# mikkleini/slam.net

Hardware: AMD Instinct MI355X
Metric: candidate-pose distance evals/sec on 2048^2 map, 1080-ray scan, 1/2/4/8 GPU (higher is better)
Workload: dtype f32 transform + u16 gather / integer sum

## Files before the change

slam.net_amd/csrc/cs_internal.h:

```cpp
#pragma once
#include "common.h"
#include <time.h>
#include <stdio.h>
#include <stdlib.h>
#include <vector>
#include <utility>

#define CS_RB_MAX 64
#define CS_RB_EXTENT_PX 128.0f
#define K1_GROUP 1024
#define K1_GROUP_BIG 2048
#define K1_RING_SLOTS 4
#define K1_GROUP_SMALL 512
#define K1_PLAN_SLOTS 8


struct k1_block_term { double a, b, m, n, nr; };

struct slamhip_cs {
    slamhip_ctx *ctx;
    float physical;
    int hs; float hscale;
    int os; float oscale;
    uint16_t *d_hole;
// ... 31 lines not shown
    bool gen_pending; uint64_t gen_seed, gen_stream;
    int shard_first, shard_count;
    float *d_ev_off;
    int *d_ev_idx;
    int cap_cand;
    float4 *d_pxcs;
    void *d_partial; size_t cap_partial;
    unsigned long long *d_k1_gmin;
    unsigned long long *d_k1_acc;
    int k1_cap_groups;
    int k1_group;
    std::vector<float> h_grp_dth, h_grp_dxy;
    std::vector<float> h_grp_lohi;
    std::vector<int> k1_tab_group, k1_tab_nc, k1_tab_nbp; int k1_uni_g0, k1_uni_ng, k1_uni_nc;
    std::vector<k1_block_term> k1_terms; std::vector<double> k1_cost, k1_lc; std::vector<int> k1_share;
    std::vector<std::pair<int, std::vector<int>>> k1_cut_cache; uint32_t k1_cut_gen, k1_cut_layout_gen;
    float k1_last_pose[3]; bool k1_last_valid;
    uint32_t k1_cut_seen_scan, k1_cut_seen_layout;
    uint32_t k1_layout_gen;
    std::vector<char> k1_cut_cand;
    std::vector<double> k1_cut_wsc;
    std::vector<double> k1_cut_wb;
    uint32_t scan_gen;
    std::vector<float> h_grp_prev; int k1_group_prev;
    bool k1_layout_dirty, k1_layout_spread; int k1_layout_budget, k1_layout_groups; float k1_layout_theta;
    bool k1_scan_dirty;
    bool k1_prelaunch;
    uint64_t pl_stats[4];
    uint32_t *d_scan_flag; uint32_t scan_flag_seq;
    bool k1_layout_stale;
    int k1_layout_target;
    float gen_sigma_xy, gen_sigma_theta;
    bool offs_theta_small;
    unsigned int *d_verify;
    int32_t *d_dist;
    uint64_t *d_key;
    uint64_t *h_key;
    float *d_grp_bounds; int cap_grp;
    float *d_best_pose;
    bool k1_want_pose;
    bool k1_pose_written;
    unsigned *k1_done_flag; unsigned k1_done_val;
    bool k1_done_armed;
    unsigned long long *k1_sig; unsigned long long k1_sig_val; bool k1_sig_armed;
    uint64_t *d_k1_ring; unsigned k1_ring_pos, k1_ring_rested;
    bool ov_op_dirty, ov_side_unjoined;
    hipEvent_t ev_ov_op, ev_ov_side;
    bool k1_ring_request;
    bool k1_ring_may_overlap;
    uint64_t *k1_ring_last;
    hipStream_t plan_stream;
    uint2 *d_plan_rec[K1_PLAN_SLOTS];
    int plan_cap_wgs;
    uint32_t plan_seq;
    uint32_t plan_count;
    uint32_t k1_launches;
    int k1_last_stream;
    uint32_t k1_cross_no[2];
    uint32_t plan_slot_user[K1_PLAN_SLOTS];
    uint8_t plan_slot_stream[K1_PLAN_SLOTS];
    uint32_t plan_inputs_after;
    uint64_t plan_stats[4];
    void *d_rep; uint32_t *h_rep; uint32_t rep_seq;
    bool k1_keep_dist;
    bool rep_dist_valid; int rep_K;
    uint32_t upload_seq;

    void *d_rays; int cap_rays;
    void *d_k2_cand;
    void *d_k2_vprof;
    int *d_k2_start;
    int *d_k2_counters;
    void *mirror_reg; size_t mirror_reg_bytes;
    bool mirror_on, mirror_pending;
    int2 *d_hole_span, *d_hole_span_snap;
    uint16_t *d_hole_shadow;
    unsigned long long *d_mirror_mask; int mirror_chunks;
    int *d_mirror_sum; int *h_mirror_sum;
    hipStream_t mirror_stream; hipEvent_t ev_snap, ev_push;
    void *mirror_dev_ptr;
    unsigned mirror_reg_flags;
    uint16_t *mirror_user; bool mirror_direct;
    uint16_t *h_mirror_stage;
    int2 *d_mirror_rows, *h_mirror_rows;
    int *d_hole_dirty;
    int64_t last_hole_pixels;
    bool hole_pixels_pending;

    uint32_t *d_o_hits[2];
    uint8_t *d_o_nohit[2];
    int obst_buf;
    bool obst_pending; int obst_pend_buf, obst_pend_max_hits;
};

int32_t cs_alloc_candidates(slamhip_cs *cs, int count);
int32_t cs_plan_drain(slamhip_cs *cs);
void    cs_plan_free(slamhip_cs *cs);
static inline void cs_plan_inputs_pending(slamhip_cs *cs) { cs->plan_inputs_after = cs->k1_launches + 1; cs->ov_op_dirty = true; }
int32_t cs_overlap_join(slamhip_cs *cs);
int32_t cs_flush_scan(slamhip_cs *cs);
int32_t cs_launch_distance(slamhip_cs *cs, int mode, const float pose[3], int count, bool want_dist, bool cand_sane,
                           uint64_t *key_dst);
#define CS_REP_WORDS 30
#define CS_REP_KEY 30
#define CS_REP_POSE 32
#define CS_REP_FLAG 63
// ... 54 lines not shown
```

slam.net_amd/csrc/distance.hip:

```cpp
#include "cs_internal.h"
#include "det_trig.h"
#include <stdlib.h>
#include <algorithm>

#define K1_THREADS 256

__device__ static inline void k1_coords(const float4 q, const float2 p, float &fx, float &fy)
{
    fx = q.x + q.z * p.x;  fx = fx - q.w * p.y;
    fy = q.y + q.w * p.x;  fy = fy + q.z * p.y;
}

template <bool SAFE>
__device__ static inline void k1_gather_global(const uint16_t *__restrict__ map, int S, const float4 q, const float2 p,
                                               uint32_t &sum, uint32_t &cnt)
{
    float fx, fy;
    k1_coords(q, p, fx, fy);
    int ix, iy;
    if (SAFE) { ix = sh_f2i(fx); iy = sh_f2i(fy); }
    else      { ix = (int)fx;    iy = (int)fy; }
    const bool ok = ((unsigned)ix < (unsigned)S) & ((unsigned)iy < (unsigned)S);
    uint32_t v = 0;
    if (ok) v = map[(size_t)iy * S + ix];
// ... 108 lines not shown
        __syncthreads();
    }
    if (w == 0) {
        for (int off = 32; off > 0; off >>= 1) {
            const unsigned long long o = __shfl_down(key, off, 64);
            key = o < key ? o : key;
        }
        if (lane == 0 && key != ~0ull) atomicMin(key_out, key);
    }
}

#define K1_KIND_SHARED 1
#define K1_KIND_GLOBAL 2
#define K1_KIND_BAND 3
#define K1_MAXP 16
#define K1_MAXR 512
#define K1_MAXBANDS 4
#define K1_MAXSTEPS (K1_MAXP * K1_MAXBANDS * 2)
static_assert(K1_MAXBANDS == 4, "the step threads split t into (piece, band) with shifts");
#define K1_TABLE_G 64
#define K1_TABLE_WGS 2048
#define K1_MAXCUT 596
#define K1_ACC_INMAP 36
#define K1_ACC_ARRIVED 50
#define K1_ZERO_OFS 0
#define K1_TILE_OFS 16

struct k1_args {
    const uint16_t *map; int S;
    const float2 *pts;
    const int4 *ray_blk;
    int n_rays;
    const float4 *pxcs;
    const float *src3;
    float bx, by, bth, scale;
    int count, n_groups;
    int budget;
    int noden;
    int nopad;
    int nosplit;
    float band_stage;
    unsigned long long *acc;
    unsigned long long *gmin;
    unsigned *done;
    const int *ev_idx;
    int32_t *dist_out;
    unsigned long long *key_out;
    unsigned *verify;
    const float *offs_flat; float *best_pose;
    unsigned long long *sig; unsigned long long sig_val;
    unsigned *done_flag; unsigned done_val;
    unsigned long long *ring_slot, *ring_reset;
    uint2 *plan_rec; uint32_t plan_seq;
    uint32_t *started; uint32_t launch_no;
    const uint32_t *scan_flag; uint32_t scan_seq;
    int n_tab_wgs, uni_g0, uni_ng, uni_nc;
    int uni_cut, tab_cut;
    const float *grp_bounds;
    struct tab_rec {
        unsigned short group;
        unsigned short nbp;
        unsigned short first, nc;
    } tab[K1_TABLE_G];
    alignas(4) unsigned char wg_pos[K1_TABLE_WGS];
    alignas(4) unsigned short cut[K1_MAXCUT];
};
static_assert(sizeof(k1_args) <= 4096, "kernel arguments are limited to 4 KB");
static_assert(sizeof(k1_args::tab_rec) == 8 && offsetof(k1_args, tab) % 8 == 0, "table records are 8-byte aligned");
#define K1_PLAN_STEPS 15
#define K1_PLAN_REC_WORDS 128

#ifdef K1_TIMES
__device__ unsigned long long g_k1_times[4096 * 16];
__device__ unsigned long long g_k1_wstart[4096 * 16];
__device__ unsigned long long g_k1_sub[4096 * 8];
#define K1_SUB(k, v) { if (threadIdx.x == 0 && blockIdx.x < 4096) g_k1_sub[blockIdx.x * 8 + (k)] += (v); }
#define K1_STAMP(k) { if (threadIdx.x == 0 && blockIdx.x < 4096) g_k1_times[blockIdx.x * 16 + (k)] = wall_clock64(); }
#else
#define K1_STAMP(k) {}
#endif

__device__ static inline unsigned k1_tile_addr(int ix, int iy, int pitch2, int kofs)
{
    unsigned t, a;
    asm("v_lshl_add_u32 %0, %1, 1, %2" : "=v"(t) : "v"(ix), "s"(kofs));
    asm("v_mad_u32_u24 %0, %1, %2, %3" : "=v"(a) : "v"(iy), "s"(pitch2), "v"(t));
    return a;
}
__device__ static inline float k1_den(int v) { return __uint_as_float(v < 0 ? (0x80000000u | (unsigned)(-v)) : (unsigned)v); }
__device__ static inline unsigned k1_tile_addr_d(float fx, float fy, float two_d, float pitch2_d, float c_d)
{
    const float g = fmaf(truncf(fy), pitch2_d, fmaf(truncf(fx), two_d, c_d));
    return __float_as_uint(g);
}
typedef __attribute__((address_space(3))) const uint16_t k1_lds_u16;
__device__ static inline uint32_t k1_lds_load(unsigned addr) { return *(k1_lds_u16 *)(size_t)addr; }
typedef __attribute__((address_space(3))) const float k1_lds_f;
__device__ static inline float2 k1_point_lds(unsigned lds_addr)
{
    k1_lds_f *p = (k1_lds_f *)(size_t)lds_addr;
    return make_float2(p[0], p[1]);
}

typedef float k1_f32x4a8 __attribute__((ext_vector_type(4), aligned(8)));
__device__ static inline float4 k1_points2_lds(unsigned lds_addr)
{
// ... 144 lines not shown
    int zv;
    asm volatile("v_mov_b32 %0, 0" : "=v"(zv));
    const int wv = __builtin_amdgcn_readfirstlane(t >> 6);
    const k1_wg_t W = k1_wg_decode(a, (int)blockIdx.x);
    const int g = W.g, nc = W.nc, nbp = W.nbp;
    if (a.ring_reset && blockIdx.x == 0 && t == 0)
        __hip_atomic_store(a.ring_reset, ~0ull, __ATOMIC_RELAXED, __HIP_MEMORY_SCOPE_AGENT);
    if (a.started && blockIdx.x == 0 && t == 0)
        __hip_atomic_store(a.started, a.launch_no, __ATOMIC_RELAXED, __HIP_MEMORY_SCOPE_SYSTEM);
    K1_STAMP(0)
#ifdef K1_TIMES
    if (t == 0 && blockIdx.x < 4096) { for (int k = 0; k < 8; k++) g_k1_sub[blockIdx.x * 8 + k] = 0; }
    if (t == 0 && blockIdx.x < 4096) { for (int k = 10; k < 16; k++) g_k1_times[blockIdx.x * 16 + k] = 0; g_k1_times[blockIdx.x * 16 + 14] = (unsigned long long)g; g_k1_times[blockIdx.x * 16 + 15] = (unsigned long long)nc; }
    if (lane == 0 && blockIdx.x < 4096) g_k1_wstart[blockIdx.x * 16 + (wv & 15)] = wall_clock64();
    if (t == 0 && blockIdx.x < 4096) {
        unsigned hw, xcc;
        asm volatile("s_getreg_b32 %0, hwreg(HW_REG_HW_ID)" : "=s"(hw));
        asm volatile("s_getreg_b32 %0, hwreg(HW_REG_XCC_ID)" : "=s"(xcc));
        g_k1_wstart[blockIdx.x * 16 + 15] = ((unsigned long long)(xcc & 15u) << 16) | ((hw >> 8) & 0xffu);
    }
#endif
    const int bp = W.bp, rlo = W.rlo, rhi = W.rhi;
    const int nrays = rhi - rlo;
    if (a.scan_flag) {
        uint32_t v = 0;
        if (wv == 0) {
            int spins = 0;
            for (;;) {
                v = __hip_atomic_load(a.scan_flag, __ATOMIC_RELAXED, __HIP_MEMORY_SCOPE_SYSTEM);
                if ((v & 0x7fffffffu) == a.scan_seq) break;
                if (++spins > (1 << 23)) { if (t == 0) atomicAdd(a.verify, 1u); v = 0x80000000u; break; }
                __builtin_amdgcn_s_sleep(32);
            }
            if (blockIdx.x == 0 && t == 0) { ((uint32_t *)a.scan_flag)[8] = (uint32_t)spins; ((uint32_t *)a.scan_flag)[9] += (uint32_t)spins; }
            if (lane == 0) s_plan_ok = (int)v;
        }
        __syncthreads();
        v = (uint32_t)s_plan_ok;
        __syncthreads();
        if (__builtin_amdgcn_readfirstlane(v) & 0x80000000u) return;
    }
    const int blk_first = a.ray_blk[rlo + zv].z;
    const int blk_last_v = a.ray_blk[rhi - 1 + zv].z;

    const bool pre = MODE == 1 && a.grp_bounds != nullptr;
    float gb[6];
    if (pre) {
#pragma unroll
        for (int k = 0; k < 6; k++) gb[k] = a.grp_bounds[8 * (size_t)g + k];
    }
    const bool planned = MODE == 1 && !LAT && pre && a.plan_rec != nullptr;
    uint2 prw = make_uint2(0u, 0u);
    if (planned && wv == 0) prw = a.plan_rec[(size_t)blockIdx.x * (K1_PLAN_REC_WORDS / 2) + lane];
    float4 q[CPL];
    float c3[CPL][3];
#pragma unroll
    for (int k = 0; k < CPL; k++) {
        const int j = g * GROUP + k * LANES + t;
        const int jc = j < count ? j : count - 1;
        if (MODE == 0) q[k] = a.pxcs[jc];
        else { c3[k][0] = a.src3[3 * jc]; c3[k][1] = a.src3[3 * jc + 1]; c3[k][2] = a.src3[3 * jc + 2]; }
    }
    int4 rinfo[RU];
    float2 rpt[RU];
#pragma unroll
    for (int u = 0; u < RU; u++) {
        const int i = u * LANES + t;
        const int r = rlo + (i < nrays ? i : 0);
        rinfo[u] = make_int4(0, 0, 0, 0); rpt[u] = make_float2(0.f, 0.f);
        if (i < nrays) { rinfo[u] = a.ray_blk[r]; rpt[u] = a.pts[r]; }
    }
    if (t == 0) { s_nsteps = 0; s_plan_ok = 0; *(unsigned *)(smem + K1_ZERO_OFS) = 0u; }
    if (MODE != 0 && !pre) {
#pragma unroll
        for (int k = 0; k < CPL; k++) q[k] = k1_candidate<MODE == 0 ? 1 : MODE, true>(c3[k], a.bx, a.by, a.bth, a.scale);
    }
#pragma unroll
    for (int u = 0; u < RU; u++) {
        const int i = u * LANES + t;
        if (i < nrays) {
            cpts[i] = rpt[u];
            if (i == 0 || rinfo[u].x == rlo + i)
                pieces[rinfo[u].z - blk_first] = make_int2(i, (rinfo[u].y < rhi ? rinfo[u].y : rhi) - (rlo + i));
        }
    }
    bool have_plan = false;
    if (planned) {
        if (wv == 0) {
            const bool okl = ((lane & 3) != 3 || prw.y == a.plan_seq) && (lane != 0 || prw.x == a.plan_seq);
            const int ns = __builtin_amdgcn_readfirstlane((int)prw.y);
            const bool ok = __builtin_amdgcn_ballot_w64(okl) == ~0ull && ns >= 0 && ns <= K1_PLAN_STEPS;
            if (lane >= 4) *(int2 *)&stepbuf[2 * lane - 8] = make_int2((int)prw.x, (int)prw.y);
            if (lane == 0 && ok) { s_plan_ok = 1; s_nsteps = ns; }
        }
        __syncthreads();
        have_plan = __builtin_amdgcn_readfirstlane(s_plan_ok) != 0;
        if (VERIFY && t == 0) atomicAdd(a.verify + (have_plan ? 5 : 6), 1u);
    }
    K1_STAMP(1)
    if (!have_plan) {
    if (pre) {
        if (wv == 0) {
            k1_bounds_from_jitter(a, gb, bnd, lane);
        }
        __syncthreads();
        K1_STAMP(2)
    } else
    {
        float lo[4] = { q[0].x, q[0].y, q[0].z, q[0].w }, hi[4] = { q[0].x, q[0].y, q[0].z, q[0].w };
#pragma unroll
        for (int k = 1; k < CPL; k++) {
            lo[0] = fminf(lo[0], q[k].x); hi[0] = fmaxf(hi[0], q[k].x); lo[1] = fminf(lo[1], q[k].y); hi[1] = fmaxf(hi[1], q[k].y);
            lo[2] = fminf(lo[2], q[k].z); hi[2] = fmaxf(hi[2], q[k].z); lo[3] = fminf(lo[3], q[k].w); hi[3] = fmaxf(hi[3], q[k].w);
        }
        const float m0 = k1_wave_redf<false>(lo[0]), m1 = k1_wave_redf<true>(hi[0]);
        const float m2 = k1_wave_redf<false>(lo[1]), m3 = k1_wave_redf<true>(hi[1]);
        const float m4 = k1_wave_redf<false>(lo[2]), m5 = k1_wave_redf<true>(hi[2]);
        const float m6 = k1_wave_redf<false>(lo[3]), m7 = k1_wave_redf<true>(hi[3]);
        if (lane == 63) {
            *(float4 *)&wred[wv][0] = make_float4(m0, m1, m2, m3);
            *(float4 *)&wred[wv][4] = make_float4(m4, m5, m6, m7);
        }
        __syncthreads();
        K1_STAMP(2)
        if (t < 8) {
            float v[NW];
#pragma unroll
            for (int w = 0; w < NW; w++) v[w] = wred[w][t];
            float x = v[0];
#pragma unroll
            for (int w = 1; w < NW; w++) x = (t & 1) ? fmaxf(x, v[w]) : fminf(x, v[w]);
            bnd[t] = x;
        }
        __syncthreads();
    }
    K1_STAMP(3)
    const int npieces = __builtin_amdgcn_readfirstlane(blk_last_v - blk_first + 1);
#define K1_PIECE_STAMP K1_STAMP(4)
#define K1_STEP_SLOT(i) (i)
#define K1_PIECE_RAY(i) (i)
#include "k1_pieces.inc"
#undef K1_PIECE_RAY
#undef K1_STEP_SLOT
#undef K1_PIECE_STAMP
    __syncthreads();
    }
#ifdef K1_TIMES
    else if (t == 0 && blockIdx.x < 4096) { const unsigned long long now_ = wall_clock64(); for (int k = 2; k <= 4; k++) g_k1_times[blockIdx.x * 16 + k] = now_; }
#endif
    const int nsteps = s_nsteps;
// ... 16 lines not shown
        {                                                                                           \
             \
             \
             \
            const int4 pa_ = *(const int4 *)&stepbuf[(step) * 8];                                   \
            const int shift_ = __builtin_amdgcn_readfirstlane(stepbuf[(step) * 8 + 4]);             \
            const int w8_ = __builtin_amdgcn_readfirstlane(pa_.z), h_ = (enable) ? __builtin_amdgcn_readfirstlane(pa_.w) : 0; \
            const int rpi = 64 >> shift_;                          \
            const int srow = lane >> shift_, scol = lane & ((1 << shift_) - 1);                     \
            const bool colok = scol < (w8_ >> 3);                                                   \
            const int cc = colok ? scol : 0;                                                        \
            const unsigned S2_ = (unsigned)S * 2u;                                                  \
            const unsigned gofs = ((unsigned)__builtin_amdgcn_readfirstlane(pa_.y) * (unsigned)S + (unsigned)__builtin_amdgcn_readfirstlane(pa_.x)) * 2u; \
            const int pitchb = w8_ << 1;                                                            \
            const int row0 = wv * rpi + srow, rstep = NW * rpi;                                     \
            unsigned vofs = gofs + (unsigned)row0 * S2_ + ((unsigned)cc << 4);                      \
            int ldsd = K1_TILE_OFS + (cc << 4) + row0 * pitchb;                                     \
            const unsigned vstep = (unsigned)rstep * S2_;                                           \
            const int lstep = rstep * pitchb;                                                       \
            _Pragma("unroll") for (int k_ = 0; k_ < PF; k_++) {                                     \
                const bool live = colok & (row0 + k_ * rstep < h_);                                 \
                if (live && K1_EXP != 3) R[k_] = *(const k1_u32x4 *)((const char *)map + vofs);    \
                dst[k_] = live ? ldsd : -1;                                                         \
                vofs += vstep; ldsd += lstep;                                                       \
            }                                                                                       \
        }
#if K1_DMA0
        {
            const int4 pa_ = *(const int4 *)&stepbuf[0];
            const int w8_ = __builtin_amdgcn_readfirstlane(pa_.z), h_ = __builtin_amdgcn_readfirstlane(pa_.w);
            const int ncols = w8_ >> 3, nunits = ncols * h_;
            const unsigned S2_ = (unsigned)S * 2u;
            const unsigned gofs = ((unsigned)__builtin_amdgcn_readfirstlane(pa_.y) * (unsigned)S + (unsigned)__builtin_amdgcn_readfirstlane(pa_.x)) * 2u;
            const float rn = 1.0f / (float)ncols;
#pragma unroll
            for (int k_ = 0; k_ < PF; k_++) {
                const int e0 = (k_ * NW + wv) * 64;
                if (e0 < nunits && K1_EXP != 3) {
                    const int e = e0 + lane;
                    const int row = (int)(((float)e + 0.5f) * rn);
                    const int col = e - row * ncols;
                    if (e < nunits)
                        __builtin_amdgcn_global_load_lds((const __attribute__((address_space(1))) void *)((const char *)map + (gofs + (unsigned)row * S2_ + ((unsigned)col << 4))),
                                                         (__attribute__((address_space(3))) void *)(smem + K1_TILE_OFS + (e0 << 4)), 16, 0, 0);
                }
            }
#pragma unroll
            for (int k_ = 0; k_ < PF; k_++) dst[k_] = -1;
        }
#else
        K1_PREFETCH(0, true)
#endif
        if (MODE != 0 && pre) {
            {
#pragma unroll
            for (int k = 0; k < CPL; k++) { if (K1_EXP == 1) q[k] = make_float4(a.bx * a.scale + c3[k][0], a.by * a.scale + c3[k][1], a.scale, c3[k][2]); else q[k] = k1_candidate<MODE == 0 ? 1 : MODE, true>(c3[k], a.bx, a.by, a.bth, a.scale); }
            }
            if (LAT) {
#pragma unroll
                for (int k = 1; k < CPL; k++)
                    if (g * GROUP + k * LANES + t < count && (__float_as_uint(q[k].z) != __float_as_uint(q[0].z) || __float_as_uint(q[k].w) != __float_as_uint(q[0].w)))
                        atomicAdd(a.verify, 1u);
            }
        }
#ifdef K1_TIMES
        const unsigned long long sclk0 = clock64();
#endif
        for (int s = 0; s < nsteps; s++) {
#ifdef K1_TIMES
            const unsigned long long ts0 = wall_clock64();
#endif
            if (K1_DMA0 && s == 0) asm volatile("s_waitcnt vmcnt(0)" ::: "memory");
            else {
            __syncthreads();
#pragma unroll
            for (int k = 0; k < PF; k++) asm volatile("" : "+v"(R[k]));
#pragma unroll
            for (int k = 0; k < PF; k++) if (dst[k] >= 0 && K1_EXP != 3) *(k1_u32x4 *)(smem + dst[k]) = R[k];
            }
            __syncthreads();
            if (s == 0) K1_STAMP(6)
#ifdef K1_TIMES
            const unsigned long long ts1 = wall_clock64();
            if (s > 0) K1_SUB(0, ts1 - ts0)
#endif
            const int4 ca = *(const int4 *)&stepbuf[s * 8], cb = *(const int4 *)&stepbuf[s * 8 + 4];
            {
                const int sn = s + 1 < nsteps ? s + 1 : s;
                K1_PREFETCH(sn, s + 1 < nsteps)
            }
#ifdef K1_TIMES
            const unsigned long long ts2 = wall_clock64();
            K1_SUB(1, ts2 - ts1) K1_SUB(3, 1ull)
#endif
            const int kind = __builtin_amdgcn_readfirstlane(cb.y);
            const int nr = __builtin_amdgcn_readfirstlane(cb.z) >> 16;
#ifdef K1_TIMES
            if (t == 0 && blockIdx.x < 4096) g_k1_times[blockIdx.x * 16 + 10 + kind] += (unsigned long long)nr;
            if (t == 0 && blockIdx.x < 4096 && s < 3)
                g_k1_sub[blockIdx.x * 8 + 5 + s] = (unsigned long long)kind | ((unsigned long long)__builtin_amdgcn_readfirstlane(ca.z) << 4) | ((unsigned long long)__builtin_amdgcn_readfirstlane(ca.w) << 16) | ((unsigned long long)nr << 32);
#endif
            const unsigned pbase = cpts_lds + (unsigned)zv + (unsigned)(__builtin_amdgcn_readfirstlane(cb.z) & 0xffff) * 8u;
            const int x0a = __builtin_amdgcn_readfirstlane(ca.x), y0 = __builtin_amdgcn_readfirstlane(ca.y);
            const int w8 = __builtin_amdgcn_readfirstlane(ca.z), h = __builtin_amdgcn_readfirstlane(ca.w);
            const int pitch2 = w8 << 1;
            const int kofs = (int)smem_lds + K1_TILE_OFS - ((y0 * w8 + x0a) << 1);
            const unsigned zaddr = smem_lds + K1_ZERO_OFS + (unsigned)zv;
// ... 251 lines not shown
        __hip_atomic_store(a.done_flag, a.done_val, __ATOMIC_RELEASE, __HIP_MEMORY_SCOPE_SYSTEM);
    }
    K1_STAMP(9)
}


__device__ static inline int k1_plan_slot(const int i) { return i <= K1_PLAN_STEPS ? i : K1_PLAN_STEPS + 1; }
template <int GROUP, int CPL>
__global__ void __launch_bounds__(64)
k1_plan(const k1_args a, const int n_wgs)
{
    constexpr int NW = 1, PF = 64;
    const int lane = threadIdx.x, wv = 0;
    const uint32_t seq = a.plan_seq;
    if ((int)blockIdx.x >= n_wgs) return;
    __shared__ __attribute__((aligned(16))) int stepbuf[(K1_PLAN_STEPS + 2) * 8];
    __shared__ int2 pieces[K1_MAXP];
    __shared__ __attribute__((aligned(16))) float bnd[8];
    __shared__ int s_nsteps;
    const int S = a.S;
    const k1_wg_t W = k1_wg_decode(a, (int)blockIdx.x);
    const int g = W.g, nbp = W.nbp, bp = W.bp, rlo = W.rlo, rhi = W.rhi, nrays = rhi - rlo;
    float gb[6];
#pragma unroll
    for (int k = 0; k < 6; k++) gb[k] = a.grp_bounds[8 * (size_t)g + k];
    const int blk_first = a.ray_blk[rlo].z, blk_last = a.ray_blk[rhi - 1].z;
    if (lane == 0) s_nsteps = 0;
    for (int i = lane; i < nrays; i += 64) {
        const int4 ri = a.ray_blk[rlo + i];
        const int pidx = ri.z - blk_first;
        if ((i == 0 || ri.x == rlo + i) && (unsigned)pidx < (unsigned)K1_MAXP) pieces[pidx] = make_int2(i, (ri.y < rhi ? ri.y : rhi) - (rlo + i));
    }
    const float2 *cpts = a.pts + rlo;
    k1_bounds_from_jitter(a, gb, bnd, lane);
    __syncthreads();
    const int npieces = min(blk_last - blk_first + 1, K1_MAXP);
#define K1_PIECE_STAMP
#define K1_STEP_SLOT(i) k1_plan_slot(i)
#define K1_PIECE_RAY(i) min(max((i), 0), nrays - 1)
#include "k1_pieces.inc"
#undef K1_PIECE_RAY
#undef K1_STEP_SLOT
#undef K1_PIECE_STAMP
    __syncthreads();
    const int nsteps = s_nsteps;
    const bool fits = nsteps <= K1_PLAN_STEPS;
    const int unit = lane >> 2, wp = lane & 3;
    uint2 w = make_uint2(0u, 0u);
    if (unit > 0 && fits && unit - 1 < nsteps) { w.x = (uint32_t)stepbuf[(unit - 1) * 8 + 2 * wp]; w.y = (uint32_t)stepbuf[(unit - 1) * 8 + 2 * wp + 1]; }
    if (lane == 0) { w.x = seq; w.y = (uint32_t)(fits ? nsteps : -1); }
    if (wp == 3) w.y = seq;
    __hip_atomic_store((unsigned long long *)(a.plan_rec + (size_t)blockIdx.x * (K1_PLAN_REC_WORDS / 2) + lane), ((unsigned long long)w.y << 32) | w.x,
                       __ATOMIC_RELAXED, __HIP_MEMORY_SCOPE_AGENT);
}

int32_t cs_overlap_join(slamhip_cs *cs)
{
    cs->ov_op_dirty = true;
    if (!cs->ov_side_unjoined) return SLAMHIP_OK;
    if (!cs->ev_ov_side) SH_HIP(hipEventCreateWithFlags(&cs->ev_ov_side, hipEventDisableTiming));
    SH_HIP(hipEventRecord(cs->ev_ov_side, cs->side_stream));
    SH_HIP(hipStreamWaitEvent(cs->ctx->stream, cs->ev_ov_side, 0));
    cs->ov_side_unjoined = false;
    cs->k1_cross_no[1] = cs->k1_launches + 1;
    return SLAMHIP_OK;
}

int32_t cs_plan_drain(slamhip_cs *cs)
{
    if (cs->plan_stream) SH_HIP(hipStreamSynchronize(cs->plan_stream));
    return SLAMHIP_OK;
}

void cs_plan_free(slamhip_cs *cs)
{
    if (cs->plan_stream) (void)hipStreamSynchronize(cs->plan_stream);
    for (int i = 0; i < K1_PLAN_SLOTS; i++) {
        (void)hipFree(cs->d_plan_rec[i]);
        cs->d_plan_rec[i] = nullptr; cs->plan_slot_user[i] = 0;
    }
    cs->plan_cap_wgs = 0;
}

int32_t cs_alloc_candidates(slamhip_cs *cs, int count)
{
    if (count <= cs->cap_cand) return SLAMHIP_OK;
    SH_TRY(cs_plan_drain(cs));
    int cap = count + (count >> 2) + 256;
    if (cs->d_ev_off) (void)hipFree(cs->d_ev_off);
    if (cs->d_ev_idx) (void)hipFree(cs->d_ev_idx);
    if (cs->d_pxcs) (void)hipFree(cs->d_pxcs);
    if (cs->d_dist) (void)hipFree(cs->d_dist);
    cs->d_ev_off = nullptr; cs->d_ev_idx = nullptr; cs->d_pxcs = nullptr; cs->d_dist = nullptr; cs->cap_cand = 0;
    SH_HIP(hipMalloc(&cs->d_ev_off, sizeof(float) * 3 * (size_t)cap));
    SH_HIP(hipMalloc(&cs->d_ev_idx, sizeof(int) * (size_t)cap));
    SH_HIP(hipMalloc(&cs->d_pxcs, sizeof(float4) * (size_t)cap));
    SH_HIP(hipMalloc(&cs->d_dist, sizeof(int32_t) * (size_t)cap));
    if (cs->d_grp_bounds) (void)hipFree(cs->d_grp_bounds);
    cs->d_grp_bounds = nullptr; cs->cap_grp = 0;
    SH_HIP(hipMalloc(&cs->d_grp_bounds, sizeof(float) * 8 * (size_t)(cap / K1_GROUP_SMALL + 2)));
    cs->cap_grp = cap / K1_GROUP_SMALL + 2;
    cs->cap_cand = cap;
    cs->rep_dist_valid = false;
    cs->shard_first = -1; cs->shard_count = -1;
    return SLAMHIP_OK;
}

static int32_t ensure_partial(slamhip_cs *cs, size_t bytes)
{
    if (bytes <= cs->cap_partial) return SLAMHIP_OK;
    if (cs->d_partial) (void)hipFree(cs->d_partial);
    cs->d_partial = nullptr; cs->cap_partial = 0;
    bytes += bytes / 4;
    SH_HIP(hipMalloc(&cs->d_partial, bytes));
    cs->cap_partial = bytes;
    return SLAMHIP_OK;
}

constexpr int K1_BAND_PARTS = 2;
constexpr float K1_BAND_STAGE = 5.0f;
constexpr double K1_CUT_CAND = 0.9;
constexpr double K1_FBAND = 1.9, K1_FGLOBAL = 3.0;
constexpr double K1_STEPCOST = 8.0;
constexpr double K1_TAILW = 1.5;

static bool k1_chunks_legal(const slamhip_cs *cs, int nc)
{
    const int R = cs->n_points, n_rb = cs->n_rb;
    const int *rb = cs->h_rb_start.data();
    if (nc < 1 || nc > R) return false;
    int b = 0;
    const int dq = R / nc, dr = R % nc;
    int rlo = 0, rem = 0;
    for (int c = 0; c < nc; c++) {
// ... 469 lines not shown
        rec.group = (unsigned short)cs->k1_tab_group[(size_t)p];
        rec.nbp = (unsigned short)cs->k1_tab_nbp[(size_t)p];
        rec.first = (unsigned short)first; rec.nc = (unsigned short)nc_p;
        if (tab_ok)
            for (int w = 0; w < nc_p; w++) a.cut[n_cut + (int)first + w] = (unsigned short)(*tcut[(size_t)p])[(size_t)(w / nbp)];
        first += (unsigned)nc_p;
    }
    if (tab_ok) a.tab_cut = n_cut;
    for (int p = 0; p < n_tab; p++)
        for (unsigned w = a.tab[p].first; w < (unsigned)a.tab[p].first + a.tab[p].nc; w++) a.wg_pos[w] = (unsigned char)p;
    a.n_tab_wgs = (int)first;
    return (int)first + a.uni_nc * cs->k1_uni_ng;
}

static int32_t k1_acc_alloc(slamhip_cs *cs, int count, int set, k1_args &a)
{
    slamhip_ctx *ctx = cs->ctx;
    if (sh_div_up(count, K1_GROUP) + 2 > cs->k1_cap_groups) {
        SH_TRY(cs_overlap_join(cs));
        if (cs->d_k1_acc) { SH_HIP(hipStreamSynchronize(ctx->stream)); (void)hipFree(cs->d_k1_acc); }
        cs->d_k1_acc = nullptr; cs->k1_cap_groups = 0;
        const int cap = sh_div_up(count, K1_GROUP) + sh_div_up(count, K1_GROUP) / 4 + 16;
        SH_HIP(hipMalloc(&cs->d_k1_acc, sizeof(unsigned long long) * 2 * (size_t)cap * K1_GROUP));
        SH_HIP(hipMemsetAsync(cs->d_k1_acc, 0, sizeof(unsigned long long) * 2 * (size_t)cap * K1_GROUP, ctx->stream));
        cs->k1_cap_groups = cap;
    }
    if (!cs->d_k1_gmin) {
        SH_HIP(hipMalloc(&cs->d_k1_gmin, 32));
        for (int s = 0; s < 2; s++) {
            SH_HIP(hipMemsetAsync((char *)cs->d_k1_gmin + 16 * s, 0xff, 8, ctx->stream));
            SH_HIP(hipMemsetAsync((char *)cs->d_k1_gmin + 16 * s + 8, 0, 8, ctx->stream));
        }
        cs->ov_op_dirty = true;
    }
    a.gmin = cs->d_k1_gmin + 2 * set; a.done = (unsigned *)((char *)cs->d_k1_gmin + 16 * set + 8);
    a.acc = cs->d_k1_acc + (size_t)set * (size_t)cs->k1_cap_groups * K1_GROUP;
    return SLAMHIP_OK;
}

static inline volatile uint32_t *k1_started_word(const slamhip_cs *cs, int s) { return (volatile uint32_t *)cs->h_key + 25 + s; }
static inline bool k1_launch_finished(const slamhip_cs *cs, int s, uint32_t no)
{
    if ((int32_t)(*k1_started_word(cs, s) - (no + 1)) >= 0) return true;
    const uint32_t x = cs->k1_cross_no[s];
    return x != 0 && (int32_t)(x - no) > 0 && (int32_t)(*k1_started_word(cs, s ^ 1) - x) >= 0;
}
static int32_t k1_plan_launch(slamhip_cs *cs, k1_args &a, int mode, int group, int n_wgs, bool lat, int s)
{
    slamhip_ctx *ctx = cs->ctx;
    static const int plan_env = (int)sh_env_int("SLAMHIP_K1_PLAN", 1);
    const uint32_t prev_no = cs->k1_launches; const int prev_s = cs->k1_last_stream;
    a.started = (uint32_t *)cs->h_key + 25 + s; a.launch_no = ++cs->k1_launches;
    cs->k1_last_stream = s;
    a.plan_rec = nullptr; a.plan_seq = 0;
    static const int plan_always = (int)sh_env_int("SLAMHIP_K1_PLAN_ALWAYS", 0);
    const bool stream_busy = plan_always || (prev_no != 0 && (int32_t)(*k1_started_word(cs, prev_s) - prev_no) < 0);
    bool plan_on = plan_env && mode == 1 && stream_busy && a.grp_bounds != nullptr && !cs->k1_prelaunch && !lat && !ctx->mail_off;
    if (plan_on && cs->plan_inputs_after != 0) {
        if ((int32_t)(*k1_started_word(cs, 0) - cs->plan_inputs_after) >= 0 || (int32_t)(*k1_started_word(cs, 1) - cs->plan_inputs_after) >= 0) cs->plan_inputs_after = 0;
        else { plan_on = false; cs->plan_stats[3]++; }
    }
    if (plan_on) {
        if (n_wgs > cs->plan_cap_wgs) {
            SH_TRY(cs_overlap_join(cs));
            SH_HIP(hipStreamSynchronize(ctx->stream));
            const int cw = std::max(cs->plan_cap_wgs, n_wgs + n_wgs / 4 + 64);
            cs_plan_free(cs);
            for (int i = 0; i < K1_PLAN_SLOTS; i++) {
                SH_HIP(hipMalloc(&cs->d_plan_rec[i], sizeof(uint32_t) * K1_PLAN_REC_WORDS * (size_t)cw));
                SH_HIP(hipMemsetAsync(cs->d_plan_rec[i], 0, sizeof(uint32_t) * K1_PLAN_REC_WORDS * (size_t)cw, cs->plan_stream));
            }
            SH_HIP(hipStreamSynchronize(cs->plan_stream));
            cs->plan_cap_wgs = cw;
        }
        const unsigned slot = cs->plan_count % K1_PLAN_SLOTS;
        const uint32_t user = cs->plan_slot_user[slot];
        const int us = cs->plan_slot_stream[slot];
        if (user != 0 && !k1_launch_finished(cs, us, user)) {
            cs->plan_stats[2]++;
            const int64_t bound_us = 1000 * (ctx->wait_timeout_ms > 0 && ctx->wait_timeout_ms < 20 ? ctx->wait_timeout_ms : 20);
            const double t0w = k1_now_us();
            for (int spins = 0; !k1_launch_finished(cs, us, user); spins++) {
                __builtin_ia32_pause();
                if ((spins & 1023) == 1023 && k1_now_us() - t0w > (double)bound_us) break;
            }
            if (!k1_launch_finished(cs, us, user)) { plan_on = false; cs->plan_stats[3]++; }
        }
    }
    if (plan_on) {
        const unsigned slot = cs->plan_count % K1_PLAN_SLOTS;
        if (++cs->plan_seq == 0) cs->plan_seq = 1;
        a.plan_rec = cs->d_plan_rec[slot]; a.plan_seq = cs->plan_seq;
        const dim3 pgrid((unsigned)n_wgs);
        if (group == K1_GROUP_BIG) hipLaunchKernelGGL((k1_plan<K1_GROUP_BIG, 4>), pgrid, dim3(64), 0, cs->plan_stream, a, n_wgs);
        else if (group == K1_GROUP_SMALL) hipLaunchKernelGGL((k1_plan<K1_GROUP_SMALL, 1>), pgrid, dim3(64), 0, cs->plan_stream, a, n_wgs);
        else hipLaunchKernelGGL((k1_plan<K1_GROUP, 2>), pgrid, dim3(64), 0, cs->plan_stream, a, n_wgs);
        SH_HIP(hipGetLastError());
        cs->plan_slot_user[slot] = a.launch_no; cs->plan_slot_stream[slot] = (uint8_t)s;
        cs->plan_count++; cs->plan_stats[0]++;
    }
    if (!plan_on) cs->plan_stats[1]++;
    return SLAMHIP_OK;
}

static void k1_search_launch(slamhip_cs *cs, const k1_args &a, int mode, int group, int n_wgs, size_t lds, bool verify, bool lat2, bool lat4, hipStream_t st)
{
    slamhip_ctx *ctx = cs->ctx;
    sh_timer t(ctx, SLAMHIP_K_CS_DISTANCE);
#define K1_LAUNCH(M, V, C, G) hipLaunchKernelGGL((k1_search_tiled<M, V, C, G>), dim3(n_wgs), dim3(G / C), lds, st, a)
#define K1_LAUNCH_LAT(C, G) hipLaunchKernelGGL((k1_search_tiled<1, false, C, G, true>), dim3(n_wgs), dim3(G / C), lds, st, a)
#define K1_LAUNCH_C(M, V) { if (group == K1_GROUP_BIG) K1_LAUNCH(M, V, 4, K1_GROUP_BIG); else if (group == K1_GROUP_SMALL) K1_LAUNCH(M, V, 1, K1_GROUP_SMALL); else K1_LAUNCH(M, V, 2, K1_GROUP); }
    if (lat2) K1_LAUNCH_LAT(2, K1_GROUP);
    else if (lat4) K1_LAUNCH_LAT(4, K1_GROUP_BIG);
    else if (verify) { if (mode == 0) K1_LAUNCH_C(0, true) else if (mode == 1) K1_LAUNCH_C(1, true) else K1_LAUNCH_C(2, true) }
    else        { if (mode == 0) K1_LAUNCH_C(0, false) else if (mode == 1) K1_LAUNCH_C(1, false) else K1_LAUNCH_C(2, false) }
#undef K1_LAUNCH_C
#undef K1_LAUNCH_LAT
#undef K1_LAUNCH
}

static int32_t k1_launch_fallback(slamhip_cs *cs, int mode, const float p[3], int count, bool sane, int32_t *dist, unsigned long long *key,
                                  unsigned long long *ring_slot, unsigned long long *ring_reset)
{
    slamhip_ctx *ctx = cs->ctx;
    const int n_rb = cs->n_rb;
    cs->k1_pose_written = false; cs->k1_done_armed = false; cs->k1_sig_armed = false;
    SH_TRY(cs_side_join(cs));
    SH_TRY(cs_overlap_join(cs));
    {
        sh_timer t(ctx, SLAMHIP_K_CS_PREP);
        const dim3 grid(sh_div_up(count, K1_THREADS));
#define K1_PREP(M) hipLaunchKernelGGL(k1_prep_pxcs<M>, grid, dim3(K1_THREADS), 0, ctx->stream, (const float *)cs->d_ev_off, \
                       p[0], p[1], p[2], cs->hscale, cs->d_pxcs, count, key)
        if (mode == 0) K1_PREP(0); else if (mode == 1) K1_PREP(1); else K1_PREP(2);
#undef K1_PREP
    }
    int bpc = (int)(((long long)sh_div_up(count, K1_THREADS) * n_rb) / 4096);
    if (bpc < 1) bpc = 1;
    if (bpc > n_rb) bpc = n_rb;
    static_assert(1023ull * CS_RB_MAX * 65535ull < (1ull << 32), "a chunk's 32-bit partial sum holds 1023 full ray blocks of 65535");
    if (bpc > 1023) bpc = 1023;
    const int n_chunks = sh_div_up(n_rb, bpc);
    SH_TRY(ensure_partial(cs, sizeof(uint2) * (size_t)n_chunks * count));
    {
        sh_timer t(ctx, SLAMHIP_K_CS_DISTANCE);
// ... 397 lines not shown
```

Measured before the change: 1.125 billion.

## Precompute candidate pose transforms in plan kernel and reuse them in search

New measurement: 866.8 million. 0.771x the previous value.

```diff
diff --git a/slam.net_amd/csrc/cs_internal.h b/slam.net_amd/csrc/cs_internal.h
--- a/slam.net_amd/csrc/cs_internal.h
+++ b/slam.net_amd/csrc/cs_internal.h
@@ -107,6 +107,8 @@
     hipStream_t plan_stream;
     uint2 *d_plan_rec[K1_PLAN_SLOTS];
     int plan_cap_wgs;
+    uint2 *d_plan_cand[K1_PLAN_SLOTS];
+    int plan_cap_cand;
     uint32_t plan_seq;
     uint32_t plan_count;
     uint32_t k1_launches;
diff --git a/slam.net_amd/csrc/distance.hip b/slam.net_amd/csrc/distance.hip
--- a/slam.net_amd/csrc/distance.hip
+++ b/slam.net_amd/csrc/distance.hip
@@ -184,6 +184,7 @@
     unsigned *done_flag; unsigned done_val;
     unsigned long long *ring_slot, *ring_reset;
     uint2 *plan_rec; uint32_t plan_seq;
+    uint2 *plan_cand;
     uint32_t *started; uint32_t launch_no;
     const uint32_t *scan_flag; uint32_t scan_seq;
     int n_tab_wgs, uni_g0, uni_ng, uni_nc;
@@ -434,14 +435,25 @@
     const bool planned = MODE == 1 && !LAT && pre && a.plan_rec != nullptr;
     uint2 prw = make_uint2(0u, 0u);
     if (planned && wv == 0) prw = a.plan_rec[(size_t)blockIdx.x * (K1_PLAN_REC_WORDS / 2) + lane];
+    const bool cand_planned = planned && a.plan_cand != nullptr;
     float4 q[CPL];
     float c3[CPL][3];
+    uint32_t cst[CPL][4];
 #pragma unroll
     for (int k = 0; k < CPL; k++) {
         const int j = g * GROUP + k * LANES + t;
         const int jc = j < count ? j : count - 1;
         if (MODE == 0) q[k] = a.pxcs[jc];
         else { c3[k][0] = a.src3[3 * jc]; c3[k][1] = a.src3[3 * jc + 1]; c3[k][2] = a.src3[3 * jc + 2]; }
+        if (cand_planned) {
+            float v[4];
+#pragma unroll
+            for (int m = 0; m < 4; m++) {
+                const unsigned long long u = __hip_atomic_load((const unsigned long long *)(a.plan_cand + (size_t)m * (size_t)count + jc), __ATOMIC_RELAXED, __HIP_MEMORY_SCOPE_WAVEFRONT);
+                v[m] = __uint_as_float((uint32_t)u); cst[k][m] = (uint32_t)(u >> 32);
+            }
+            q[k] = make_float4(v[0], v[1], v[2], v[3]);
+        }
     }
     int4 rinfo[RU];
     float2 rpt[RU];
@@ -467,7 +479,14 @@
         }
     }
     bool have_plan = false;
+    bool cand_ok = false;
     if (planned) {
+        if (cand_planned) {
+            bool okl = true;
+#pragma unroll
+            for (int k = 0; k < CPL; k++) okl = okl && cst[k][0] == a.plan_seq && cst[k][1] == a.plan_seq && cst[k][2] == a.plan_seq && cst[k][3] == a.plan_seq;
+            cand_ok = __builtin_amdgcn_ballot_w64(okl) == ~0ull;
+        }
         if (wv == 0) {
             const bool okl = ((lane & 3) != 3 || prw.y == a.plan_seq) && (lane != 0 || prw.x == a.plan_seq);
             const int ns = __builtin_amdgcn_readfirstlane((int)prw.y);
@@ -478,6 +497,8 @@
         __syncthreads();
         have_plan = __builtin_amdgcn_readfirstlane(s_plan_ok) != 0;
         if (VERIFY && t == 0) atomicAdd(a.verify + (have_plan ? 5 : 6), 1u);
+        cand_ok = cand_ok && have_plan;
+        if (VERIFY && lane == 0 && cand_ok) atomicAdd(a.verify + 7, 1u);
     }
     K1_STAMP(1)
     if (!have_plan) {
@@ -600,7 +621,7 @@
         K1_PREFETCH(0, true)
 #endif
         if (MODE != 0 && pre) {
-            {
+            if (!cand_ok) {
 #pragma unroll
             for (int k = 0; k < CPL; k++) { if (K1_EXP == 1) q[k] = make_float4(a.bx * a.scale + c3[k][0], a.by * a.scale + c3[k][1], a.scale, c3[k][2]); else q[k] = k1_candidate<MODE == 0 ? 1 : MODE, true>(c3[k], a.bx, a.by, a.bth, a.scale); }
             }
@@ -958,6 +979,18 @@
     if (wp == 3) w.y = seq;
     __hip_atomic_store((unsigned long long *)(a.plan_rec + (size_t)blockIdx.x * (K1_PLAN_REC_WORDS / 2) + lane), ((unsigned long long)w.y << 32) | w.x,
                        __ATOMIC_RELAXED, __HIP_MEMORY_SCOPE_AGENT);
+    if (a.plan_cand != nullptr && W.chunk == 0) {
+        const int j1 = min((g + 1) * GROUP, a.count);
+        for (int j = g * GROUP + lane; j < j1; j += 64) {
+            const float c3[3] = { a.src3[3 * j], a.src3[3 * j + 1], a.src3[3 * j + 2] };
+            const float4 q = k1_candidate<1, true>(c3, a.bx, a.by, a.bth, a.scale);
+            const float v[4] = { q.x, q.y, q.z, q.w };
+#pragma unroll
+            for (int m = 0; m < 4; m++)
+                __hip_atomic_store((unsigned long long *)(a.plan_cand + (size_t)m * (size_t)a.count + j), ((unsigned long long)seq << 32) | __float_as_uint(v[m]),
+                                   __ATOMIC_RELAXED, __HIP_MEMORY_SCOPE_AGENT);
+        }
+    }
 }
 
 int32_t cs_overlap_join(slamhip_cs *cs)
@@ -983,9 +1016,10 @@
     if (cs->plan_stream) (void)hipStreamSynchronize(cs->plan_stream);
     for (int i = 0; i < K1_PLAN_SLOTS; i++) {
         (void)hipFree(cs->d_plan_rec[i]);
-        cs->d_plan_rec[i] = nullptr; cs->plan_slot_user[i] = 0;
-    }
-    cs->plan_cap_wgs = 0;
+        (void)hipFree(cs->d_plan_cand[i]);
+        cs->d_plan_rec[i] = nullptr; cs->d_plan_cand[i] = nullptr; cs->plan_slot_user[i] = 0;
+    }
+    cs->plan_cap_wgs = 0; cs->plan_cap_cand = 0;
 }
 
 int32_t cs_alloc_candidates(slamhip_cs *cs, int count)
@@ -1561,7 +1595,7 @@
     const uint32_t prev_no = cs->k1_launches; const int prev_s = cs->k1_last_stream;
     a.started = (uint32_t *)cs->h_key + 25 + s; a.launch_no = ++cs->k1_launches;
     cs->k1_last_stream = s;
-    a.plan_rec = nullptr; a.plan_seq = 0;
+    a.plan_rec = nullptr; a.plan_seq = 0; a.plan_cand = nullptr;
     static const int plan_always = (int)sh_env_int("SLAMHIP_K1_PLAN_ALWAYS", 0);
     const bool stream_busy = plan_always || (prev_no != 0 && (int32_t)(*k1_started_word(cs, prev_s) - prev_no) < 0);
     bool plan_on = plan_env && mode == 1 && stream_busy && a.grp_bounds != nullptr && !cs->k1_prelaunch && !lat && !ctx->mail_off;
@@ -1569,18 +1603,24 @@
         if ((int32_t)(*k1_started_word(cs, 0) - cs->plan_inputs_after) >= 0 || (int32_t)(*k1_started_word(cs, 1) - cs->plan_inputs_after) >= 0) cs->plan_inputs_after = 0;
         else { plan_on = false; cs->plan_stats[3]++; }
     }
+    static const int plan_cand_env = (int)sh_env_int("SLAMHIP_K1_PLAN_CAND", 1);
     if (plan_on) {
-        if (n_wgs > cs->plan_cap_wgs) {
+        if (n_wgs > cs->plan_cap_wgs || (plan_cand_env && a.count > cs->plan_cap_cand)) {
             SH_TRY(cs_overlap_join(cs));
             SH_HIP(hipStreamSynchronize(ctx->stream));
-            const int cw = std::max(cs->plan_cap_wgs, n_wgs + n_wgs / 4 + 64);
+            const int cw = n_wgs > cs->plan_cap_wgs ? n_wgs + n_wgs / 4 + 64 : cs->plan_cap_wgs;
+            const int cc = !plan_cand_env ? 0 : a.count > cs->plan_cap_cand ? a.count + a.count / 4 + 256 : cs->plan_cap_cand;
             cs_plan_free(cs);
             for (int i = 0; i < K1_PLAN_SLOTS; i++) {
                 SH_HIP(hipMalloc(&cs->d_plan_rec[i], sizeof(uint32_t) * K1_PLAN_REC_WORDS * (size_t)cw));
                 SH_HIP(hipMemsetAsync(cs->d_plan_rec[i], 0, sizeof(uint32_t) * K1_PLAN_REC_WORDS * (size_t)cw, cs->plan_stream));
+                if (cc > 0) {
+                    SH_HIP(hipMalloc(&cs->d_plan_cand[i], sizeof(uint2) * 4 * (size_t)cc));
+                    SH_HIP(hipMemsetAsync(cs->d_plan_cand[i], 0, sizeof(uint2) * 4 * (size_t)cc, cs->plan_stream));
+                }
             }
             SH_HIP(hipStreamSynchronize(cs->plan_stream));
-            cs->plan_cap_wgs = cw;
+            cs->plan_cap_wgs = cw; cs->plan_cap_cand = cc;
         }
         const unsigned slot = cs->plan_count % K1_PLAN_SLOTS;
         const uint32_t user = cs->plan_slot_user[slot];
@@ -1600,6 +1640,7 @@
         const unsigned slot = cs->plan_count % K1_PLAN_SLOTS;
         if (++cs->plan_seq == 0) cs->plan_seq = 1;
         a.plan_rec = cs->d_plan_rec[slot]; a.plan_seq = cs->plan_seq;
+        a.plan_cand = plan_cand_env ? cs->d_plan_cand[slot] : nullptr;
         const dim3 pgrid((unsigned)n_wgs);
         if (group == K1_GROUP_BIG) hipLaunchKernelGGL((k1_plan<K1_GROUP_BIG, 4>), pgrid, dim3(64), 0, cs->plan_stream, a, n_wgs);
         else if (group == K1_GROUP_SMALL) hipLaunchKernelGGL((k1_plan<K1_GROUP_SMALL, 1>), pgrid, dim3(64), 0, cs->plan_stream, a, n_wgs);
```
